# voidstrike/FPSG

Hardware: AMD Instinct MI355X
Metric: episodes/sec (+ Chamfer-kernel HBM GB/s in roofline.hbm), 2048-pt clouds, 224x224 images; episode = fwd + Chamfer + bwd, step = E episodes + all-reduce + Adam (higher is better)
Workload: dtype f32

## Files before the change

fpsg_amd/_hip.py:

```python
from __future__ import annotations

import ctypes
import os
import threading

import torch

_HERE = os.path.dirname(os.path.abspath(__file__))
LIB_PATH = os.environ.get("FPSG_HIP_LIB") or os.path.join(_HERE, "libfpsg_hip.so")

_c_f32p = ctypes.c_void_p
_c_i32p = ctypes.c_void_p
_c_int = ctypes.c_int
_c_stream = ctypes.c_void_p

SIGNATURES = {
    "fpsg_version": [],
    "fpsg_last_error": [],
    "fpsg_stream_threshold_bytes": [],
    "fpsg_chamfer_fwd": [_c_f32p, _c_f32p, _c_int, _c_int, _c_int,
                         _c_f32p, _c_i32p, _c_f32p, _c_i32p, _c_stream],
    "fpsg_chamfer_bwd": [_c_f32p, _c_f32p, _c_i32p, _c_i32p, _c_f32p, _c_f32p,
                         _c_int, _c_int, _c_int, _c_f32p, _c_f32p, _c_stream],
    "fpsg_chamfer_losses": [_c_f32p, _c_f32p, _c_int, _c_int, _c_int, _c_int, ctypes.c_float, ctypes.c_float, _c_f32p,
# ... 73 lines not shown
                             _c_f32p, _c_f32p, _c_f32p, _c_f32p, _c_stream],
    "fpsg_bn_act_bwd_parts": [_c_f32p, _c_f32p, _c_f32p, _c_f32p, _c_int, _c_int, _c_int, _c_int, _c_int,
                        ctypes.c_float, _c_f32p, _c_f32p, _c_f32p, _c_f32p, _c_f32p, _c_f32p, _c_f32p, _c_int, _c_stream],
    "fpsg_bn_pool_workspace_floats": [_c_int, _c_int, _c_int, _c_int],
    "fpsg_bn_act_pool_fwd": [_c_f32p, _c_f32p, _c_f32p, _c_f32p, _c_f32p, _c_f32p, ctypes.c_float, _c_int, _c_int, _c_int, _c_int,
                             _c_int, ctypes.c_float, _c_int, ctypes.c_float, _c_f32p, _c_f32p, _c_f32p, _c_f32p,
                             _c_f32p, _c_f32p, _c_int, _c_stream],
    "fpsg_bn_act_pool_bwd": [_c_f32p, _c_f32p, _c_f32p, _c_f32p, _c_int, _c_int, _c_int, _c_int, _c_int, _c_int,
                             ctypes.c_float, _c_f32p, _c_f32p, _c_f32p, _c_f32p, _c_f32p, _c_f32p, _c_stream],
    "fpsg_bn_max_workspace_floats": [_c_int, _c_int, _c_int],
    "fpsg_bn_max_dz_offset": [_c_int, _c_int, _c_int],
    "fpsg_bn_act_max_fwd": [_c_f32p, _c_f32p, _c_f32p, _c_f32p, _c_f32p, _c_f32p, ctypes.c_float, _c_int, _c_int, _c_int, _c_int,
                            ctypes.c_float, _c_int, ctypes.c_float, _c_f32p, _c_i32p, _c_f32p, _c_f32p, _c_f32p,
                            _c_f32p, _c_stream],
    "fpsg_bn_act_max_bwd": [_c_f32p, _c_f32p, _c_f32p, _c_i32p, _c_f32p, _c_int, _c_int, _c_int, _c_int, _c_int,
                            ctypes.c_float, _c_f32p, _c_f32p, _c_f32p, _c_f32p, _c_f32p, _c_f32p, _c_stream],
    "fpsg_max_bwd_prep": [_c_f32p, _c_f32p, _c_f32p, _c_f32p, _c_f32p, _c_f32p, _c_int, _c_int, _c_int, _c_int, _c_f32p, _c_f32p,
                          _c_f32p, _c_f32p, _c_stream],
    "fpsg_max_bwd_dw": [_c_f32p, _c_f32p, _c_f32p, _c_f32p, _c_f32p, _c_int, _c_int, _c_int, _c_f32p, _c_stream],
    "fpsg_max_bwd_gather": [_c_f32p, _c_f32p, _c_i32p, _c_int, _c_int, _c_int, _c_int, _c_f32p, _c_f32p, _c_stream],
    "fpsg_max_bwd_scatter": [_c_f32p, _c_f32p, _c_f32p, _c_f32p, _c_i32p, _c_f32p, _c_int, _c_int, _c_int, _c_int, _c_f32p,
                             _c_stream],
    "fpsg_max_bwd_scatter_workspace_floats": [_c_int, _c_int, _c_int],
    "fpsg_bn_act_max_bwd_coef": [_c_f32p, _c_f32p, _c_f32p, _c_i32p, _c_f32p, _c_int, _c_int, _c_int, _c_int, _c_int,
                                 ctypes.c_float, _c_f32p, _c_f32p, _c_f32p, _c_f32p, _c_stream],
    "fpsg_wino_input_transform": [_c_int, _c_f32p, _c_int, _c_int, _c_int, _c_int, _c_f32p, ctypes.c_long, _c_stream],
    "fpsg_wino_output_transform": [_c_int, _c_f32p, _c_int, _c_int, _c_int, _c_int, _c_f32p, ctypes.c_long, _c_stream],
    "fpsg_wino_stats_parts": [_c_int, _c_int, _c_int, _c_int],
    "fpsg_wino_output_transform_stats": [_c_int, _c_f32p, _c_int, _c_int, _c_int, _c_int, _c_f32p, _c_f32p, _c_f32p,
                                         ctypes.c_long, _c_stream],
    "fpsg_wino_grad_output_transform": [_c_int, _c_f32p, _c_int, _c_int, _c_int, _c_int, _c_f32p, ctypes.c_long, _c_stream],
    "fpsg_wino_grad_transforms": [_c_int, _c_f32p, _c_int, _c_int, _c_int, _c_int, _c_f32p, _c_f32p, ctypes.c_long, _c_stream],
    "fpsg_wino_filter_transform": [_c_int, _c_f32p, _c_int, _c_int, _c_int, _c_f32p, _c_stream],
    "fpsg_wino_output_transform_bwd_stats": [_c_int, _c_f32p, _c_int, _c_int, _c_int, _c_int, _c_f32p, _c_f32p, _c_f32p,
                                             _c_f32p, _c_f32p, ctypes.c_long, _c_stream],
    "fpsg_wino_filter_transform_batch": [ctypes.c_void_p, _c_int, ctypes.c_long, _c_stream],
    "fpsg_wino_filter_grad_transform": [_c_int, _c_f32p, _c_int, _c_int, _c_f32p, _c_stream],
    "fpsg_wino_conv_fused": [_c_f32p, _c_f32p, _c_int, _c_int, _c_int, _c_int, _c_int, _c_f32p, _c_stream],
    "fpsg_wino_input_transform_act": [_c_int, _c_f32p, _c_f32p, _c_f32p, _c_int, _c_int, _c_int, _c_int, _c_f32p, ctypes.c_long,
                                      _c_stream],
    "fpsg_wino_conv_fused_act": [_c_f32p, _c_f32p, _c_f32p, _c_f32p, _c_int, _c_int, _c_int, _c_int, _c_int, _c_f32p,
                                 _c_stream],
    "fpsg_wino_dw_fused_workspace_floats": [_c_int, _c_int, _c_int, _c_int],
    "fpsg_wino_dw_fused": [_c_f32p, _c_f32p, _c_f32p, _c_f32p, _c_int, _c_int, _c_int, _c_int, _c_int, _c_f32p, _c_f32p,
                           _c_stream],
    "fpsg_wino_conv_fused_parts": [_c_int, _c_int, _c_int, _c_int],
    "fpsg_wino_conv_fused_stats": [_c_f32p, _c_f32p, _c_f32p, _c_f32p, _c_int, _c_int, _c_int, _c_int, _c_int, _c_f32p,
                                   _c_f32p, _c_f32p, _c_stream],
    "fpsg_bn_stats": [_c_f32p, _c_f32p, _c_f32p, _c_f32p, _c_f32p, _c_f32p, ctypes.c_float, _c_int, _c_int, _c_int, _c_int,
                      ctypes.c_float, _c_f32p, _c_f32p, _c_f32p, _c_f32p, _c_f32p, _c_int, _c_stream],
    "fpsg_conv_first_dw_workspace_floats": [_c_int, _c_int, _c_int],
    "fpsg_conv_first_parts": [_c_int, _c_int, _c_int],
    "fpsg_conv_first_fwd": [_c_f32p, _c_f32p, _c_int, _c_int, _c_int, _c_int, _c_int, _c_f32p, _c_f32p, _c_f32p, _c_stream],
    "fpsg_conv_first_dw": [_c_f32p, _c_f32p, _c_int, _c_int, _c_int, _c_int, _c_int, _c_f32p, _c_f32p, _c_stream],
    "fpsg_conv_first_dw_fold": [_c_f32p, _c_f32p, _c_f32p, _c_f32p, _c_f32p, _c_f32p, _c_int, _c_int, _c_int, _c_int, _c_int,
                                _c_f32p, _c_f32p, _c_stream],
    "fpsg_adam_step": [_c_f32p, _c_f32p, _c_f32p, _c_f32p, ctypes.c_size_t, ctypes.c_float, ctypes.c_float,
                       ctypes.c_float, ctypes.c_float, _c_int, ctypes.c_float, _c_stream],
    "fpsg_flat_accumulate_segments": [_c_f32p, ctypes.c_void_p, ctypes.c_void_p, _c_int, ctypes.c_size_t, _c_int, _c_stream],
    "fpsg_flat_accumulate_tables": [_c_f32p, ctypes.c_void_p, ctypes.c_void_p, _c_int, _c_int, ctypes.c_size_t, _c_int,
                                    _c_stream],
    "fpsg_adam_step_segments": [_c_f32p, ctypes.c_void_p, ctypes.c_void_p, _c_int, _c_f32p, _c_f32p, ctypes.c_size_t,
                                ctypes.c_float, ctypes.c_float, ctypes.c_float, ctypes.c_float, _c_int, ctypes.c_float,
                                _c_stream],
    "fpsg_grad_norm_workspace_bytes": [ctypes.c_size_t],
    "fpsg_grad_clip_scale": [_c_f32p, ctypes.c_size_t, ctypes.c_float, ctypes.c_float, ctypes.c_void_p, ctypes.c_size_t,
# ... 180 lines not shown
```

fpsg_amd/csrc/winograd.hip:

```cpp
#include "fpsg_common.h"

namespace fpsg {
namespace {

template <bool NT>
__device__ __forceinline__ void stream_store(float* p, float v) {
  if constexpr (NT) __builtin_nontemporal_store(v, p);
  else *p = v;
}
template <bool NT>
__device__ __forceinline__ float stream_load(const float* p) {
  if constexpr (NT) return __builtin_nontemporal_load(p);
  else return *p;
}

constexpr int kWinoThreads = 256;

template <int M> struct Wino;

template <> struct Wino<2> {
  static constexpr int A = 4;
  static __device__ __forceinline__ void in(const float (&d)[4], float (&t)[4]) {
    t[0] = d[0] - d[2]; t[1] = d[1] + d[2]; t[2] = d[2] - d[1]; t[3] = d[1] - d[3];
  }
// ... 318 lines not shown
      v2 lo = {0.0f, 0.0f}, hi = {0.0f, 0.0f};
      if (M * ti.th + i < H) {
        lo = *reinterpret_cast<const v2*>(yp + (size_t)i * W);
        if (M * ti.tw + 2 < W) hi = *reinterpret_cast<const v2*>(yp + (size_t)i * W + 2);
      }
      yv[i][0] = lo[0]; yv[i][1] = lo[1]; yv[i][M - 2] = hi[0]; yv[i][M - 1] = hi[1];
    } else {
      const vin v = *reinterpret_cast<const vin*>(yp + (size_t)i * W);
#pragma unroll
      for (int j = 0; j < M; ++j) yv[i][j] = v[j];
    }
  }
  float r[M][A];
#pragma unroll
  for (int j = 0; j < M; ++j) {
    float col[M];
#pragma unroll
    for (int i = 0; i < M; ++i) col[i] = yv[i][j];
    Wino<M>::gout(col, r[j]);
  }
  const size_t plane = (size_t)K * Ps;
  float* mp = dM + (size_t)k * Ps + p;
#pragma unroll
  for (int i = 0; i < A; ++i) {
    float row[M], o[A];
#pragma unroll
    for (int j = 0; j < M; ++j) row[j] = r[j][i];
    Wino<M>::gout(row, o);
#pragma unroll
    for (int j = 0; j < A; ++j) stream_store<NT>(mp + (size_t)(A * i + j) * plane, o[j]);
  }
}

template <int M>
__device__ __forceinline__ void wino_filter_one(const float* __restrict__ w, int K, int C, int flip, float* __restrict__ U,
                                                long e) {
  constexpr int A = Wino<M>::A;
  const int k = flip ? (int)(e % K) : (int)(e / C), c = flip ? (int)(e / K) : (int)(e % C);
  const float* g = w + ((size_t)k * C + c) * 9;
  float t[3][A];
#pragma unroll
  for (int j = 0; j < 3; ++j) {
    float col[3];
#pragma unroll
    for (int i = 0; i < 3; ++i) col[i] = flip ? g[(2 - i) * 3 + (2 - j)] : g[i * 3 + j];
    Wino<M>::flt(col, t[j]);
  }
  const size_t plane = (size_t)K * C;
  float* up = U + (flip ? (size_t)c * K + k : (size_t)k * C + c);
#pragma unroll
  for (int i = 0; i < A; ++i) {
    float row[3], o[A];
#pragma unroll
    for (int j = 0; j < 3; ++j) row[j] = t[j][i];
    Wino<M>::flt(row, o);
#pragma unroll
    for (int j = 0; j < A; ++j) up[(size_t)(A * i + j) * plane] = o[j];
  }
}

template <int M>
__global__ void wino_filter_kernel(const float* __restrict__ w, int K, int C, int flip, float* __restrict__ U) {
  const long e = (long)blockIdx.x * blockDim.x + threadIdx.x;
  if (e >= (long)K * C) return;
  wino_filter_one<M>(w, K, C, flip, U, e);
}
// ... 210 lines not shown
                                          fpsg_stream_t stream) {
  using namespace fpsg;
  FPSG_REQUIRE(m == 2 || m == 4, FPSG_E_SHAPE, "fpsg_wino_filter_transform: m must be 2 or 4 (got %d)", m);
  FPSG_REQUIRE(K > 0 && C > 0, FPSG_E_SHAPE, "fpsg_wino_filter_transform: K,C must be positive (got %d,%d)", K, C);
  FPSG_REQUIRE_PTR(w); FPSG_REQUIRE_PTR(U);
  const long n = (long)K * C;
  dim3 grid((unsigned)((n + 255) / 256));
  if (m == 2) hipLaunchKernelGGL(wino_filter_kernel<2>, grid, dim3(256), 0, static_cast<hipStream_t>(stream), w, K, C, flip_transpose, U);
  else hipLaunchKernelGGL(wino_filter_kernel<4>, grid, dim3(256), 0, static_cast<hipStream_t>(stream), w, K, C, flip_transpose, U);
  return launch_status("fpsg_wino_filter_transform");
}

extern "C" int fpsg_wino_filter_transform_batch(const int64_t* jobs, int n_jobs, long total_blocks, fpsg_stream_t stream) {
  using namespace fpsg;
  FPSG_REQUIRE(n_jobs > 0 && total_blocks > 0 && total_blocks < (1L << 31), FPSG_E_SHAPE,
               "fpsg_wino_filter_transform_batch: n_jobs and total_blocks must be positive (got %d, %ld)", n_jobs, total_blocks);
  FPSG_REQUIRE_PTR(jobs);
  hipLaunchKernelGGL(wino_filter_batch_kernel, dim3((unsigned)total_blocks), dim3(256), 0, static_cast<hipStream_t>(stream),
                     reinterpret_cast<const long long*>(jobs), n_jobs);
  return launch_status("fpsg_wino_filter_transform_batch");
}

extern "C" int fpsg_wino_filter_grad_transform(int m, const float* dU, int K, int C, float* dw, fpsg_stream_t stream) {
  using namespace fpsg;
  FPSG_REQUIRE(m == 2 || m == 4, FPSG_E_SHAPE, "fpsg_wino_filter_grad_transform: m must be 2 or 4 (got %d)", m);
  FPSG_REQUIRE(K > 0 && C > 0, FPSG_E_SHAPE, "fpsg_wino_filter_grad_transform: K,C must be positive (got %d,%d)", K, C);
  FPSG_REQUIRE_PTR(dU); FPSG_REQUIRE_PTR(dw);
  const long n = (long)K * C;
  dim3 grid((unsigned)((n + 255) / 256));
  if (m == 2) hipLaunchKernelGGL(wino_filter_grad_kernel<2>, grid, dim3(256), 0, static_cast<hipStream_t>(stream), dU, K, C, dw);
  else hipLaunchKernelGGL(wino_filter_grad_kernel<4>, grid, dim3(256), 0, static_cast<hipStream_t>(stream), dU, K, C, dw);
  return launch_status("fpsg_wino_filter_grad_transform");
}
```

fpsg_amd/winograd.py:

```python
from __future__ import annotations

import os

import torch

from . import _hip, gemm_split
from .bn_counters import count_batch

MIN_CHANNELS_M4 = 64
MIN_CHANNELS_M2 = 128
MIN_WIDE_CHANNELS_M2 = 256


def enabled() -> bool:
    return os.environ.get("FPSG_WINOGRAD", "1") != "0"


def _eligible_layer(conv: torch.nn.Conv2d, H: int, W: int) -> bool:
    def is_(v, want):
        return v == want or v == (want, want)
    return (enabled() and is_(conv.kernel_size, 3) and is_(conv.stride, 1) and is_(conv.padding, 1) and is_(conv.dilation, 1)
            and conv.groups == 1 and conv.padding_mode == "zeros" and H % 2 == 0 and W % 2 == 0
            and _wide_enough(conv.in_channels, conv.out_channels, tile_size(H, W)))

# ... 213 lines not shown
    if dev.type != "cuda" or torch.cuda.is_current_stream_capturing():
        return chan, 0
    opt = lambda t: _hip.ptr(t) if t is not None else None
    with torch.cuda.device(dev):
        _call("fpsg_bn_stats", _hip.ptr(chan), None, opt(gamma), opt(beta), _hip.ptr(running_mean), _hip.ptr(running_var),
              0.0, 1, C, 1, 0, float(eps), _hip.ptr(chan), None, None, None, None, 0,
              torch.cuda.current_stream(dev).cuda_stream)
    cache[key] = chan
    return chan, 2


def _filter(m, w, flip):
    key = (w.data_ptr(), m, bool(flip))
    capturing = w.is_cuda and torch.cuda.is_current_stream_capturing()
    banked = _bank.lookup(key, w, capturing)
    if banked is not None:
        return banked
    cache = _frozen_cache
    if cache is not None and capturing:
        cache = _ReadOnlyView(cache) if _frozen_constant else None
    if cache is not None and key in cache:
        return cache[key]
    K, C = w.shape[0], w.shape[1]
    a2 = (m + 2) ** 2
    U = torch.empty((a2, C, K) if flip else (a2, K, C), dtype=torch.float32, device=w.device)
    _call("fpsg_wino_filter_transform", m, _hip.ptr(w), K, C, 1 if flip else 0, _hip.ptr(U), _hip.stream_of(w))
    if cache is not None and not capturing:
        cache[key] = U
        if filter_bank_enabled():
            _bank.register(key, w.detach(), U)
    return U


def row_stride(P: int) -> int:
    a = int(os.environ.get("FPSG_WINO_ROW_ALIGN", "32"))
    if a < 1 or a > 1024:
        raise ValueError(f"FPSG_WINO_ROW_ALIGN must be in 1 .. 1024 (got {a})")
    return (P + a - 1) // a * a


def _ldp(T, N, H, W, m):
    if not T.is_contiguous() or T.shape[2] < N * _tiles(H, W, m):
        raise ValueError(f"transform-domain tensor {tuple(T.shape)} must be contiguous with at least "
                         f"{N * _tiles(H, W, m)} columns")
    return T.shape[2]


def _input(m, x):
    N, C, H, W = x.shape
    Ps = row_stride(N * _tiles(H, W, m))
    V = torch.empty(((m + 2) ** 2, C, Ps), dtype=torch.float32, device=x.device)
    _call("fpsg_wino_input_transform", m, _hip.ptr(x), N, C, H, W, _hip.ptr(V), Ps, _hip.stream_of(x))
    return V


def stats_enabled() -> bool:
    return os.environ.get("FPSG_CONV_STATS", "1") != "0"


_BN_SMALL_MAX = 16384


def bwd_stats_enabled() -> bool:
    return os.environ.get("FPSG_CONV_BWD_STATS", "1") != "0"


# ... 30 lines not shown
    opt = lambda t: _hip.ptr(t) if t is not None else None
    _call("fpsg_wino_conv_fused_stats", _hip.ptr(x), opt(chan), opt(pre_bias), _hip.ptr(U), N, C, K, H, W, _hip.ptr(y),
          opt(stats_bias), _hip.ptr(parts), _hip.stream_of(x))
    return y, parts


def _fused(x, U):
    N, C, H, W = x.shape
    K = U.shape[1]
    y = torch.empty((N, K, H, W), dtype=torch.float32, device=x.device)
    _call("fpsg_wino_conv_fused", _hip.ptr(x), _hip.ptr(U), N, C, K, H, W, _hip.ptr(y), _hip.stream_of(x))
    return y


def _grad_output(m, gy):
    N, K, H, W = gy.shape
    Ps = row_stride(N * _tiles(H, W, m))
    dM = torch.empty(((m + 2) ** 2, K, Ps), dtype=torch.float32, device=gy.device)
    _call("fpsg_wino_grad_output_transform", m, _hip.ptr(gy), N, K, H, W, _hip.ptr(dM), Ps, _hip.stream_of(gy))
    return dM


def grad_transforms_enabled() -> bool:
    return os.environ.get("FPSG_GRAD_TRANSFORMS", "1") != "0"


def _grad_transforms(m, gy):
    N, K, H, W = gy.shape
    Ps = row_stride(N * _tiles(H, W, m))
    V = torch.empty(((m + 2) ** 2, K, Ps), dtype=torch.float32, device=gy.device)
    dM = torch.empty_like(V)
    _call("fpsg_wino_grad_transforms", m, _hip.ptr(gy), N, K, H, W, _hip.ptr(V), _hip.ptr(dM), Ps, _hip.stream_of(gy))
    return V, dM


def _filter_grad(m, dU, like):
    gw = torch.empty_like(like)
    _call("fpsg_wino_filter_grad_transform", m, _hip.ptr(dU), like.shape[0], like.shape[1], _hip.ptr(gw),
          _hip.stream_of(dU))
    return gw


class _Conv3x3(torch.autograd.Function):

    @staticmethod
    def forward(ctx, x, w, m, stats_bias=None, want_parts=False):
        ctx.set_materialize_grads(False)
        x, w = x.contiguous(), w.contiguous()
        N, C, H, W = x.shape
        K = w.shape[0]
        parts = None
        with torch.cuda.device(x.device):
            if _can_fuse(m, C, K, N * H * W, H, W):
                if want_parts:
                    y, parts = _fused_stats(x, None, None, _filter(m, w, False), stats_bias)
                else:
                    y = _fused(x, _filter(m, w, False))
                keep, kept_is_v = x, False
            else:
                V = _input(m, x)
                Mt = _bmm(_filter(m, w, False), V)
                if want_parts:
                    y, parts = _output(m, Mt, N, H, W, stats_bias, True)
                else:
                    y = _output(m, Mt, N, H, W)
                keep, kept_is_v = V, True
        ctx.save_for_backward(keep if ctx.needs_input_grad[1] else None, w)
        ctx.dims = (N, C, H, W, m, kept_is_v)
        if not want_parts:
            return y
        if parts is not None:
            ctx.mark_non_differentiable(parts)
        return y, parts

    @staticmethod
    def backward(ctx, gy, _gparts=None):
        if gy is None:
            return None, None, None, None, None
        kept, w = ctx.saved_tensors
        N, C, H, W, m, kept_is_v = ctx.dims
        K = w.shape[0]
        gy = gy.contiguous()
        gx = gw = None
        with torch.cuda.device(gy.device):
            fuse_dx = _can_fuse(m, K, C, N * H * W, H, W)
            fuse_dw = not kept_is_v and _can_fuse_dw(m, C, K, N, H, W)
            Vg = dM = None
            if (ctx.needs_input_grad[0] and ctx.needs_input_grad[1] and not fuse_dx and not fuse_dw
                    and grad_transforms_enabled()):
                Vg, dM = _grad_transforms(m, gy)
            if ctx.needs_input_grad[0]:
                if fuse_dx:
                    gx = _fused(gy, _filter(m, w, True))
                else:
                    gx = _output(m, _bmm(_filter(m, w, True), Vg if Vg is not None else _input(m, gy)), N, H, W)
                    Vg = None
            if ctx.needs_input_grad[1]:
                if fuse_dw:
                    gw = _filter_grad(m, _fused_dw(kept, None, None, gy), w)
                else:
                    V = kept if kept_is_v else _input(m, kept)
                    gw = _filter_grad(m, _bmm_nt(dM if dM is not None else _grad_output(m, gy), V), w)
        return gx, gw, None, None, None


def _input_act(m, x, chan, pre_bias):
    N, C, H, W = x.shape
    Ps = row_stride(N * _tiles(H, W, m))
    V = torch.empty(((m + 2) ** 2, C, Ps), dtype=torch.float32, device=x.device)
    _call("fpsg_wino_input_transform_act", m, _hip.ptr(x), _hip.ptr(chan), _hip.ptr(pre_bias) if pre_bias is not None else None,
          N, C, H, W, _hip.ptr(V), Ps, _hip.stream_of(x))
    return V


def _fused_act(x, chan, pre_bias, U):
    N, C, H, W = x.shape
    K = U.shape[1]
    y = torch.empty((N, K, H, W), dtype=torch.float32, device=x.device)
    _call("fpsg_wino_conv_fused_act", _hip.ptr(x), _hip.ptr(chan), _hip.ptr(pre_bias) if pre_bias is not None else None,
          _hip.ptr(U), N, C, K, H, W, _hip.ptr(y), _hip.stream_of(x))
    return y


def fold_enabled() -> bool:
    return os.environ.get("FPSG_BN_FOLD", "1") != "0"
# ... 29 lines not shown
                    out = _fused_act(y, chan, pre_bias, _filter(m, w, False))
                V = None
            else:
                V = _input_act(m, y, chan, pre_bias)
                Mt = _bmm(_filter(m, w, False), V)
                if want_parts:
                    out, out_parts = _output(m, Mt, N, H, W, stats_bias, True)
                else:
                    out = _output(m, Mt, N, H, W)
        ctx.save_for_backward(y, chan, pre_bias, w, V if ctx.needs_input_grad[9] else None)
        ctx.cfg = (N, C, H, W, m, bool(training), gamma is not None, beta is not None)
        if not want_parts:
            return out
        if out_parts is not None:
            ctx.mark_non_differentiable(out_parts)
        return out, out_parts

    @staticmethod
    def backward(ctx, gout, _gparts=None):
        if gout is None:
            return (None,) * 14
        y, chan, pre_bias, w, V = ctx.saved_tensors
        N, C, H, W, m, training, has_g, has_b = ctx.cfg
        K = w.shape[0]
        lib = _hip.load()
        dev = y.device
        gout = gout.contiguous()
        gw = None
        with torch.cuda.device(dev):
            bwd_parts = None
            fuse_dx = _can_fuse(m, K, C, N * H * W, H, W)
            fuse_dw = V is None and _can_fuse_dw(m, C, K, N, H, W)
            Vg = dM = None
            if ctx.needs_input_grad[9] and not fuse_dx and not fuse_dw and grad_transforms_enabled():
                Vg, dM = _grad_transforms(m, gout)
            if fuse_dx:
                ga = _fused(gout, _filter(m, w, True))
            elif bwd_stats_enabled() and N * H * W > _BN_SMALL_MAX:
                ga, bwd_parts = _output_bwd_stats(m, _bmm(_filter(m, w, True), Vg if Vg is not None else _input(m, gout)),
                                                  N, H, W, y, pre_bias, chan)
            else:
                ga = _output(m, _bmm(_filter(m, w, True), Vg if Vg is not None else _input(m, gout)), N, H, W)
            Vg = None
            if ctx.needs_input_grad[9]:
                if fuse_dw:
                    gw = _filter_grad(m, _fused_dw(y, chan, pre_bias, gout), w)
                else:
                    if V is None:
                        V = _input_act(m, y, chan, pre_bias)
                    gw = _filter_grad(m, _bmm_nt(dM if dM is not None else _grad_output(m, gout), V), w)
            want_dpb = pre_bias is not None and ctx.needs_input_grad[1]
            dy = torch.empty_like(y)
            dgamma = torch.empty((C,), dtype=torch.float32, device=dev)
            dbeta = torch.empty((C,), dtype=torch.float32, device=dev)
            dpb = torch.empty((C,), dtype=torch.float32, device=dev) if want_dpb else None
            coef = torch.empty((3, C), dtype=torch.float32, device=dev)
            ws = torch.empty((lib.fpsg_bn_workspace_floats(N, C, H * W),), dtype=torch.float32, device=dev)
            if bwd_parts is not None:
                _call("fpsg_bn_act_bwd_parts", _hip.ptr(y), _hip.ptr(pre_bias) if pre_bias is not None else None,
                      _hip.ptr(ga), _hip.ptr(chan), N, C, H * W, 1 if training else 0, 1, 0.0, _hip.ptr(dy),
                      _hip.ptr(dgamma), _hip.ptr(dbeta), _hip.ptr(dpb) if want_dpb else None, _hip.ptr(coef),
                      _hip.ptr(ws), _hip.ptr(bwd_parts), bwd_parts.shape[1], _hip.stream_of(y))
            else:
                _call("fpsg_bn_act_bwd", _hip.ptr(y), _hip.ptr(pre_bias) if pre_bias is not None else None, _hip.ptr(ga),
                      _hip.ptr(chan), N, C, H * W, 1 if training else 0, 1, 0.0, _hip.ptr(dy), _hip.ptr(dgamma),
                      _hip.ptr(dbeta), _hip.ptr(dpb) if want_dpb else None, _hip.ptr(coef), _hip.ptr(ws), _hip.stream_of(y))
        return (dy, dpb, dgamma if has_g else None, dbeta if has_b else None, None, None, None, None, None, gw, None,
                None, None, None)

# ... 129 lines not shown
```

include/fpsg_hip.h:

```cpp
#ifndef FPSG_HIP_H
#define FPSG_HIP_H

#include <stddef.h>
#include <stdint.h>

#ifdef __cplusplus
extern "C" {
#endif

typedef void* fpsg_stream_t;

#define FPSG_ABI_VERSION 1

#define FPSG_E_NULL   (-1)
#define FPSG_E_SHAPE  (-2)
#define FPSG_E_ALIGN  (-3)
#define FPSG_E_LIMIT  (-4)

int         fpsg_version(void);
const char* fpsg_last_error(void);
size_t      fpsg_stream_threshold_bytes(void);

int fpsg_chamfer_fwd(const float* xyz1, const float* xyz2, int B, int N, int M,
                     float* dist1, int32_t* idx1, float* dist2, int32_t* idx2,
// ... 235 lines not shown
int fpsg_bn_act_max_bwd(const float* x, const float* pre_bias, const float* gout, const int32_t* idx,
                        const float* chan, int N, int C, int L, int training, int act, float slope, float* dx,
                        float* dgamma, float* dbeta, float* dpre_bias, float* coef, float* ws, fpsg_stream_t stream);
int fpsg_bn_act_max_bwd_coef(const float* x, const float* pre_bias, const float* gout, const int32_t* idx,
                             const float* chan, int N, int C, int L, int training, int act, float slope,
                             float* dgamma, float* dbeta, float* coef, float* ws, fpsg_stream_t stream);

int fpsg_max_bwd_gather(const float* a, const float* dz, const int32_t* idx, int B, int K, int C, int L, float* S,
                        float* spart , fpsg_stream_t stream);
int fpsg_max_bwd_prep(const float* W, const float* coef, const float* pre_bias, const float* mean, const float* dz,
                      const float* spart, int B, int K, int C, int L, float* Wk, float* u, float* dpre_bias, float* s,
                      fpsg_stream_t stream);
int fpsg_max_bwd_dw(const float* S, const float* WG, const float* coef, const float* pre_bias, const float* s, int B,
                    int K, int C, float* dw, fpsg_stream_t stream);
size_t fpsg_max_bwd_scatter_workspace_floats(int B, int C, int L);
int fpsg_max_bwd_scatter(float* da, const float* W, const float* k1, const float* dz, const int32_t* idx, const float* v,
                         int B, int K, int C, int L, float* ws, fpsg_stream_t stream);


int fpsg_wino_input_transform(int m, const float* x, int N, int C, int H, int W, float* V, long ldp,
                              fpsg_stream_t stream);
int fpsg_wino_output_transform(int m, const float* M, int N, int K, int H, int W, float* y, long ldp,
                               fpsg_stream_t stream);
int fpsg_wino_stats_parts(int m, int N, int H, int W);
int fpsg_wino_output_transform_stats(int m, const float* M, int N, int K, int H, int W, float* y, const float* bias,
                                     float* parts, long ldp, fpsg_stream_t stream);
int fpsg_wino_output_transform_bwd_stats(int m, const float* M, int N, int K, int H, int W, float* y,
                                         const float* xpre, const float* pre_bias, const float* chan,
                                         float* parts, long ldp, fpsg_stream_t stream);
int fpsg_wino_grad_output_transform(int m, const float* dy, int N, int K, int H, int W, float* dM, long ldp,
                                    fpsg_stream_t stream);
int fpsg_wino_grad_transforms(int m, const float* dy, int N, int K, int H, int W, float* V, float* dM, long ldp,
                              fpsg_stream_t stream);
int fpsg_wino_filter_transform(int m, const float* w, int K, int C, int flip_transpose, float* U,
                               fpsg_stream_t stream);
int fpsg_wino_filter_transform_batch(const int64_t* jobs, int n_jobs, long total_blocks, fpsg_stream_t stream);
int fpsg_wino_filter_grad_transform(int m, const float* dU, int K, int C, float* dw, fpsg_stream_t stream);

size_t fpsg_gemm_split_workspace_floats(int batch, int M, int N, int K, int transB, int variant);
int fpsg_gemm_split(const float* A, const float* B, float* C, int batch, int M, int N, int K, int lda, int ldb, int ldc,
                    long sA, long sB, long sC, int transB, int variant, float* ws, size_t ws_floats,
                    fpsg_stream_t stream);

size_t fpsg_gemm_split_packed_a_bytes(int batch, int M, int K, int variant);
int fpsg_gemm_split_pack_a(const float* A, int batch, int M, int K, int lda, long sA, int variant, void* Ap,
                           fpsg_stream_t stream);
int fpsg_gemm_split_nn_packed(const void* Ap, const float* B, float* C, int batch, int M, int N, int K, int ldb, int ldc,
                              long sB, long sC, int variant, fpsg_stream_t stream);

int fpsg_gemm_split_nn_persistent(const void* Ap, const float* B, float* C, int batch, int M, int N, int K, int ldb, int ldc,
                                  long sB, long sC, int variant, fpsg_stream_t stream);

int fpsg_gemm_f32_nn(const float* A, const float* B, float* C, int batch, int M, int N, int K, int lda, int ldb, int ldc,
                     long sA, long sB, long sC, int variant, fpsg_stream_t stream);

int fpsg_wino_conv_fused(const float* x, const float* U, int N, int C, int K, int H, int W, float* y,
                         fpsg_stream_t stream);

int fpsg_wino_conv_fused_parts(int N, int K, int H, int W);
int fpsg_wino_conv_fused_stats(const float* x, const float* chan, const float* pre_bias, const float* U, int N, int C,
                               int K, int H, int W, float* y, const float* out_bias, float* parts, fpsg_stream_t stream);

size_t fpsg_wino_dw_fused_workspace_floats(int N, int K, int H, int W);
int fpsg_wino_dw_fused(const float* x, const float* chan, const float* pre_bias, const float* dy, int N, int C, int K,
                       int H, int W, float* dU, float* ws, fpsg_stream_t stream);

// ... 129 lines not shown
```

Baseline: 45.85.

## Compute Winograd conv input gradient via adjoint of input transform

For F(4x4,3x3) Winograd convolutions, the data gradient is now computed as the transpose of the forward: the output gradient is grad-output-transformed (dM), multiplied by a transposed filter transform, then scattered back through the adjoint of the input transform. Overlapping tile contributions are handled with neighbour loads and wave shuffles, and a variant fuses the BN/activation backward statistics. This avoids re-running the input transform on the output gradient and the separate flipped-filter path, reusing dM that dw already needs. It applies only for large tensors (>=64MB transform buffer) and adds a more complex halo-handling kernel.

Measured after the change: 46.40 (median of 2 runs). No clear change (+1.2%).

```diff
diff --git a/fpsg_amd/_hip.py b/fpsg_amd/_hip.py
--- a/fpsg_amd/_hip.py
+++ b/fpsg_amd/_hip.py
@@ -129,6 +129,10 @@
     "fpsg_wino_grad_output_transform": [_c_int, _c_f32p, _c_int, _c_int, _c_int, _c_int, _c_f32p, ctypes.c_long, _c_stream],
     "fpsg_wino_grad_transforms": [_c_int, _c_f32p, _c_int, _c_int, _c_int, _c_int, _c_f32p, _c_f32p, ctypes.c_long, _c_stream],
     "fpsg_wino_filter_transform": [_c_int, _c_f32p, _c_int, _c_int, _c_int, _c_f32p, _c_stream],
+    "fpsg_wino_input_adjoint_parts": [_c_int, _c_int, _c_int],
+    "fpsg_wino_input_adjoint": [_c_int, _c_f32p, _c_int, _c_int, _c_int, _c_int, ctypes.c_long, _c_f32p, _c_stream],
+    "fpsg_wino_input_adjoint_bwd_stats": [_c_int, _c_f32p, _c_int, _c_int, _c_int, _c_int, ctypes.c_long, _c_f32p, _c_f32p,
+                                          _c_f32p, _c_f32p, _c_f32p, _c_int, _c_stream],
     "fpsg_wino_output_transform_bwd_stats": [_c_int, _c_f32p, _c_int, _c_int, _c_int, _c_int, _c_f32p, _c_f32p, _c_f32p,
                                              _c_f32p, _c_f32p, ctypes.c_long, _c_stream],
     "fpsg_wino_filter_transform_batch": [ctypes.c_void_p, _c_int, ctypes.c_long, _c_stream],
diff --git a/fpsg_amd/csrc/winograd.hip b/fpsg_amd/csrc/winograd.hip
--- a/fpsg_amd/csrc/winograd.hip
+++ b/fpsg_amd/csrc/winograd.hip
@@ -374,6 +374,147 @@
   }
 }
 
+__device__ __forceinline__ void wino4_in_t(const float (&v)[6], float (&o)[6]) {
+  const float p12 = v[1] + v[2], m12 = v[1] - v[2], p34 = v[3] + v[4], m34 = v[3] - v[4];
+  o[0] = 4.0f * v[0];
+  o[1] = fma_rn(-4.0f, m12, fma_rn(-2.0f, m34, 4.0f * v[5]));
+  o[2] = fma_rn(-5.0f, v[0], fma_rn(-4.0f, p12, -p34));
+  o[3] = fma_rn(2.0f, m34, fma_rn(-5.0f, v[5], m12));
+  o[4] = (v[0] + p12) + p34;
+  o[5] = v[5];
+}
+
+template <bool NT, bool BWD>
+__global__ __launch_bounds__(kWinoThreads) void wino_input_adjoint_kernel(const float* __restrict__ dV, int C, int H, int W,
+                                                                           int Th, int Tw, long P, long Ps,
+                                                                           float* __restrict__ dx,
+                                                                           const float* __restrict__ xpre,
+                                                                           const float* __restrict__ pre_bias,
+                                                                           const float* __restrict__ chan,
+                                                                           float* __restrict__ parts) {
+  typedef float v4 __attribute__((ext_vector_type(4)));
+  const long p_raw = (long)blockIdx.x * kWinoThreads + threadIdx.x;
+  const bool live = p_raw < P;
+  const long p = live ? p_raw : P - 1;
+  const int c = blockIdx.y;
+  const TileIndex ti = tile_of(p, Th, Tw);
+  const int lane = threadIdx.x & (kWave - 1);
+  const bool has_left = ti.tw > 0, has_right = ti.tw < Tw - 1, has_up = ti.th > 0, has_down = ti.th < Th - 1;
+  const bool left_lane = has_left && lane > 0;
+  const bool right_lane = has_right && lane < kWave - 1;
+  const size_t plane = (size_t)C * Ps;
+  const float* vp = dV + (size_t)c * Ps + p;
+  const long up_off = has_up ? -(long)Tw : 0, dn_off = has_down ? (long)Tw : 0;
+  float own[36], up[6], dn[6];
+#pragma unroll
+  for (int q = 0; q < 36; ++q) own[q] = stream_load<NT>(vp + (size_t)q * plane);
+#pragma unroll
+  for (int j = 0; j < 6; ++j) {
+    up[j] = stream_load<NT>(vp + up_off + (size_t)(30 + j) * plane);
+    dn[j] = stream_load<NT>(vp + dn_off + (size_t)j * plane);
+  }
+  float el[8], er[8];
+#pragma unroll
+  for (int i = 0; i < 8; ++i) el[i] = er[i] = 0.0f;
+  if (has_left && !left_lane) {
+#pragma unroll
+    for (int i = 0; i < 6; ++i) el[i] = stream_load<NT>(vp - 1 + (size_t)(6 * i + 5) * plane);
+    el[6] = stream_load<NT>(vp - 1 + up_off + (size_t)35 * plane);
+    el[7] = stream_load<NT>(vp - 1 + dn_off + (size_t)5 * plane);
+  }
+  if (has_right && !right_lane) {
+#pragma unroll
+    for (int i = 0; i < 6; ++i) er[i] = stream_load<NT>(vp + 1 + (size_t)(6 * i) * plane);
+    er[6] = stream_load<NT>(vp + 1 + up_off + (size_t)30 * plane);
+    er[7] = stream_load<NT>(vp + 1 + dn_off);
+  }
+  const size_t yoff = (((size_t)ti.n * C + c) * H + 4 * ti.th) * W + 4 * ti.tw;
+  v4 xrow[4];
+  float b = 0.0f, sc = 0.0f, sh = 0.0f, mu = 0.0f, rs = 0.0f;
+  if constexpr (BWD) {
+    b = pre_bias ? pre_bias[c] : 0.0f;
+    sc = chan[c]; sh = chan[C + c]; mu = chan[2 * C + c]; rs = chan[3 * C + c];
+#pragma unroll
+    for (int i = 0; i < 4; ++i) xrow[i] = *reinterpret_cast<const v4*>(xpre + yoff + (size_t)i * W);
+  }
+  float t[6][6];
+#pragma unroll
+  for (int j = 0; j < 6; ++j) {
+    float col[6];
+#pragma unroll
+    for (int i = 0; i < 6; ++i) col[i] = own[6 * i + j];
+    wino4_in_t(col, t[j]);
+  }
+  float R[4][6];
+#pragma unroll
+  for (int i = 0; i < 4; ++i) {
+    float row[6];
+#pragma unroll
+    for (int j = 0; j < 6; ++j) row[j] = t[j][1 + i];
+    wino4_in_t(row, R[i]);
+  }
+  float u[6], d4[6], d[6];
+  wino4_in_t(up, u);
+#pragma unroll
+  for (int j = 0; j < 6; ++j) d4[j] = 4.0f * dn[j];
+  wino4_in_t(d4, d);
+#pragma unroll
+  for (int j = 0; j < 6; ++j) {
+    R[0][j] += has_up ? u[j] : 0.0f;
+    R[3][j] += has_down ? d[j] : 0.0f;
+  }
+  float lt[6], rt[6], L[4], Rr[4];
+  {
+    float lcol[6], rcol[6];
+#pragma unroll
+    for (int i = 0; i < 6; ++i) { lcol[i] = el[i]; rcol[i] = er[i]; }
+    wino4_in_t(lcol, lt);
+    wino4_in_t(rcol, rt);
+  }
+#pragma unroll
+  for (int i = 0; i < 4; ++i) { L[i] = lt[1 + i]; Rr[i] = 4.0f * rt[1 + i]; }
+  L[0] += has_up ? el[6] : 0.0f;
+  L[3] += has_down ? 4.0f * el[7] : 0.0f;
+  Rr[0] += has_up ? 4.0f * er[6] : 0.0f;
+  Rr[3] += has_down ? 4.0f * (4.0f * er[7]) : 0.0f;
+  float* yp = dx + yoff;
+  float a0 = 0.0f, a1 = 0.0f;
+#pragma unroll
+  for (int i = 0; i < 4; ++i) {
+    float lft = __shfl_up(R[i][5], 1, kWave);
+    float rgt = __shfl_down(R[i][0], 1, kWave);
+    if (!left_lane) lft = has_left ? L[i] : 0.0f;
+    if (!right_lane) rgt = has_right ? Rr[i] : 0.0f;
+    const float o[4] = {R[i][1] + lft, R[i][2], R[i][3], R[i][4] + rgt};
+    if (live) *reinterpret_cast<v4*>(yp + (size_t)i * W) = (v4){o[0], o[1], o[2], o[3]};
+    if constexpr (BWD) {
+#pragma unroll
+      for (int j = 0; j < 4; ++j) {
+        const float xv = xrow[i][j] + b;
+        const float dz = (live && fma_rn(xv, sc, sh) > 0.0f) ? o[j] : 0.0f;
+        a0 += dz;
+        a1 = fma_rn(dz, (xv - mu) * rs, a1);
+      }
+    }
+  }
+  if constexpr (BWD) {
+    __shared__ float red[2 * (kWinoThreads / kWave)];
+    a0 = wave_sum(a0);
+    a1 = wave_sum(a1);
+    const int wave = threadIdx.x / kWave;
+    if (lane == 0) { red[2 * wave] = a0; red[2 * wave + 1] = a1; }
+    __syncthreads();
+    if (threadIdx.x == 0) {
+      float t0 = red[0], t1 = red[1];
+#pragma unroll
+      for (int w = 1; w < kWinoThreads / kWave; ++w) { t0 += red[2 * w]; t1 += red[2 * w + 1]; }
+      float* out = parts + ((size_t)c * gridDim.x + blockIdx.x) * 2;
+      out[0] = t0;
+      out[1] = t1;
+    }
+  }
+}
+
 template <int M>
 __device__ __forceinline__ void wino_filter_one(const float* __restrict__ w, int K, int C, int flip, float* __restrict__ U,
                                                 long e) {
@@ -650,3 +791,67 @@
   else hipLaunchKernelGGL(wino_filter_grad_kernel<4>, grid, dim3(256), 0, static_cast<hipStream_t>(stream), dU, K, C, dw);
   return launch_status("fpsg_wino_filter_grad_transform");
 }
+
+namespace fpsg {
+namespace {
+
+int check_adjoint(const char* fn, int m, int N, int C, int H, int W, long ldp) {
+  FPSG_REQUIRE(m == 4, FPSG_E_SHAPE, "%s: m must be 4 (got %d)", fn, m);
+  FPSG_REQUIRE(N > 0 && C > 0 && H > 0 && W > 0 && H % 4 == 0 && W % 4 == 0, FPSG_E_SHAPE,
+               "%s: N,C positive and H,W positive multiples of 4 (got %d,%d,%d,%d)", fn, N, C, H, W);
+  const long P = (long)N * (H / 4) * (W / 4);
+  FPSG_REQUIRE(C <= 65535 && (P + kWinoThreads - 1) / kWinoThreads < (1L << 31), FPSG_E_LIMIT,
+               "%s: C=%d or tile count %ld beyond the grid limits", fn, C, P);
+  FPSG_REQUIRE(ldp == 0 || ldp >= P, FPSG_E_SHAPE, "%s: row stride %ld must be 0 or at least the %ld tiles", fn, ldp, P);
+  return 0;
+}
+
+}
+}
+
+extern "C" int fpsg_wino_input_adjoint_parts(int N, int H, int W) {
+  if (N <= 0 || H <= 0 || W <= 0 || H % 4 || W % 4) return 0;
+  const long P = (long)N * (H / 4) * (W / 4);
+  return (int)((P + fpsg::kWinoThreads - 1) / fpsg::kWinoThreads);
+}
+
+extern "C" int fpsg_wino_input_adjoint(int m, const float* dV, int N, int C, int H, int W, long ldp, float* dx,
+    fpsg_stream_t stream) {
+  using namespace fpsg;
+  int rc = check_adjoint("fpsg_wino_input_adjoint", m, N, C, H, W, ldp);
+  if (rc) return rc;
+  FPSG_REQUIRE_PTR(dV); FPSG_REQUIRE_PTR(dx);
+  FPSG_REQUIRE((reinterpret_cast<uintptr_t>(dx) & 15) == 0, FPSG_E_ALIGN, "fpsg_wino_input_adjoint: dx must be 16-byte aligned");
+  const int Th = H / 4, Tw = W / 4;
+  const long P = (long)N * Th * Tw;
+  const long Ps = ldp ? ldp : P;
+  dim3 grid((unsigned)((P + kWinoThreads - 1) / kWinoThreads), C);
+  hipStream_t hs = static_cast<hipStream_t>(stream);
+  if (beyond_cache((size_t)36 * C * Ps * sizeof(float))) hipLaunchKernelGGL((wino_input_adjoint_kernel<true, false>), grid, dim3(kWinoThreads), 0, hs, dV, C, H, W, Th, Tw, P, Ps, dx, nullptr, nullptr, nullptr, nullptr);
+  else hipLaunchKernelGGL((wino_input_adjoint_kernel<false, false>), grid, dim3(kWinoThreads), 0, hs, dV, C, H, W, Th, Tw, P, Ps, dx, nullptr, nullptr, nullptr, nullptr);
+  return launch_status("fpsg_wino_input_adjoint");
+}
+
+extern "C" int fpsg_wino_input_adjoint_bwd_stats(int m, const float* dV, int N, int C, int H, int W, long ldp, float* dx,
+                                                 const float* y, const float* pre_bias, const float* chan, float* parts,
+                                                 int n_parts,
+    fpsg_stream_t stream) {
+  using namespace fpsg;
+  int rc = check_adjoint("fpsg_wino_input_adjoint_bwd_stats", m, N, C, H, W, ldp);
+  if (rc) return rc;
+  FPSG_REQUIRE_PTR(dV); FPSG_REQUIRE_PTR(dx); FPSG_REQUIRE_PTR(y); FPSG_REQUIRE_PTR(chan); FPSG_REQUIRE_PTR(parts);
+  FPSG_REQUIRE(((reinterpret_cast<uintptr_t>(dx) | reinterpret_cast<uintptr_t>(y)) & 15) == 0, FPSG_E_ALIGN,
+               "fpsg_wino_input_adjoint_bwd_stats: dx and y must be 16-byte aligned");
+  FPSG_REQUIRE(!misaligned4(pre_bias), FPSG_E_ALIGN, "fpsg_wino_input_adjoint_bwd_stats: pre_bias not 4-byte aligned");
+  const int Th = H / 4, Tw = W / 4;
+  const long P = (long)N * Th * Tw;
+  const long Ps = ldp ? ldp : P;
+  FPSG_REQUIRE(n_parts == fpsg_wino_input_adjoint_parts(N, H, W), FPSG_E_SHAPE,
+               "fpsg_wino_input_adjoint_bwd_stats: n_parts %d must be fpsg_wino_input_adjoint_parts(N,H,W) = %d", n_parts,
+               fpsg_wino_input_adjoint_parts(N, H, W));
+  dim3 grid((unsigned)((P + kWinoThreads - 1) / kWinoThreads), C);
+  hipStream_t hs = static_cast<hipStream_t>(stream);
+  if (beyond_cache((size_t)36 * C * Ps * sizeof(float))) hipLaunchKernelGGL((wino_input_adjoint_kernel<true, true>), grid, dim3(kWinoThreads), 0, hs, dV, C, H, W, Th, Tw, P, Ps, dx, y, pre_bias, chan, parts);
+  else hipLaunchKernelGGL((wino_input_adjoint_kernel<false, true>), grid, dim3(kWinoThreads), 0, hs, dV, C, H, W, Th, Tw, P, Ps, dx, y, pre_bias, chan, parts);
+  return launch_status("fpsg_wino_input_adjoint_bwd_stats");
+}
diff --git a/fpsg_amd/winograd.py b/fpsg_amd/winograd.py
--- a/fpsg_amd/winograd.py
+++ b/fpsg_amd/winograd.py
@@ -269,6 +269,23 @@
     return U
 
 
+def _filter_t(m, w):
+    key = (w.data_ptr(), m, "t")
+    capturing = w.is_cuda and torch.cuda.is_current_stream_capturing()
+    cache = _frozen_cache
+    if cache is not None and capturing:
+        cache = _ReadOnlyView(cache) if _frozen_constant else None
+    if cache is not None and key in cache:
+        return cache[key]
+    K, C = w.shape[0], w.shape[1]
+    wt = w.transpose(0, 1).contiguous()
+    U = torch.empty(((m + 2) ** 2, C, K), dtype=torch.float32, device=w.device)
+    _call("fpsg_wino_filter_transform", m, _hip.ptr(wt), C, K, 0, _hip.ptr(U), _hip.stream_of(w))
+    if cache is not None and not capturing:
+        cache[key] = U
+    return U
+
+
 def row_stride(P: int) -> int:
     a = int(os.environ.get("FPSG_WINO_ROW_ALIGN", "32"))
     if a < 1 or a > 1024:
@@ -365,6 +382,34 @@
     dM = torch.empty_like(V)
     _call("fpsg_wino_grad_transforms", m, _hip.ptr(gy), N, K, H, W, _hip.ptr(V), _hip.ptr(dM), Ps, _hip.stream_of(gy))
     return V, dM
+
+
+MIN_ADJOINT_BYTES = 64 << 20
+
+
+def adjoint_mode() -> str:
+    return os.environ.get("FPSG_WINO_ADJOINT", "auto")
+
+
+def _adjoint_applies(m: int, K: int, N: int, H: int, W: int) -> bool:
+    mode = adjoint_mode()
+    if mode == "0" or m != 4 or H % 4 or W % 4:
+        return False
+    return mode == "1" or 36 * K * row_stride(N * _tiles(H, W, 4)) * 4 >= MIN_ADJOINT_BYTES
+
+
+def _input_adjoint(m, dV, N, H, W, xpre=None, pre_bias=None, chan=None):
+    C = dV.shape[1]
+    ga = torch.empty((N, C, H, W), dtype=torch.float32, device=dV.device)
+    if xpre is None:
+        _call("fpsg_wino_input_adjoint", m, _hip.ptr(dV), N, C, H, W, _ldp(dV, N, H, W, m), _hip.ptr(ga), _hip.stream_of(dV))
+        return ga
+    S = _hip.load().fpsg_wino_input_adjoint_parts(N, H, W)
+    parts = torch.empty((C, S, 2), dtype=torch.float32, device=dV.device)
+    _call("fpsg_wino_input_adjoint_bwd_stats", m, _hip.ptr(dV), N, C, H, W, _ldp(dV, N, H, W, m), _hip.ptr(ga),
+          _hip.ptr(xpre), _hip.ptr(pre_bias) if pre_bias is not None else None, _hip.ptr(chan), _hip.ptr(parts), S,
+          _hip.stream_of(dV))
+    return ga, parts
 
 
 def _filter_grad(m, dU, like):
@@ -419,11 +464,16 @@
             fuse_dx = _can_fuse(m, K, C, N * H * W, H, W)
             fuse_dw = not kept_is_v and _can_fuse_dw(m, C, K, N, H, W)
             Vg = dM = None
-            if (ctx.needs_input_grad[0] and ctx.needs_input_grad[1] and not fuse_dx and not fuse_dw
-                    and grad_transforms_enabled()):
+            both = ctx.needs_input_grad[0] and ctx.needs_input_grad[1] and not fuse_dx and not fuse_dw
+            adjoint = both and _adjoint_applies(m, K, N, H, W)
+            if adjoint:
+                dM = _grad_output(m, gy)
+            elif both and grad_transforms_enabled():
                 Vg, dM = _grad_transforms(m, gy)
             if ctx.needs_input_grad[0]:
-                if fuse_dx:
+                if adjoint:
+                    gx = _input_adjoint(m, _bmm(_filter_t(m, w), dM), N, H, W)
+                elif fuse_dx:
                     gx = _fused(gy, _filter(m, w, True))
                 else:
                     gx = _output(m, _bmm(_filter(m, w, True), Vg if Vg is not None else _input(m, gy)), N, H, W)
@@ -519,9 +569,20 @@
             fuse_dx = _can_fuse(m, K, C, N * H * W, H, W)
             fuse_dw = V is None and _can_fuse_dw(m, C, K, N, H, W)
             Vg = dM = None
-            if ctx.needs_input_grad[9] and not fuse_dx and not fuse_dw and grad_transforms_enabled():
+            both = ctx.needs_input_grad[9] and not fuse_dx and not fuse_dw
+            adjoint = both and _adjoint_applies(m, K, N, H, W)
+            if adjoint:
+                dM = _grad_output(m, gout)
+            elif both and grad_transforms_enabled():
                 Vg, dM = _grad_transforms(m, gout)
-            if fuse_dx:
+            if adjoint:
+                dV = _bmm(_filter_t(m, w), dM)
+                if bwd_stats_enabled() and N * H * W > _BN_SMALL_MAX:
+                    ga, bwd_parts = _input_adjoint(m, dV, N, H, W, y, pre_bias, chan)
+                else:
+                    ga = _input_adjoint(m, dV, N, H, W)
+                dV = None
+            elif fuse_dx:
                 ga = _fused(gout, _filter(m, w, True))
             elif bwd_stats_enabled() and N * H * W > _BN_SMALL_MAX:
                 ga, bwd_parts = _output_bwd_stats(m, _bmm(_filter(m, w, True), Vg if Vg is not None else _input(m, gout)),
diff --git a/include/fpsg_hip.h b/include/fpsg_hip.h
--- a/include/fpsg_hip.h
+++ b/include/fpsg_hip.h
@@ -291,6 +291,12 @@
                                     fpsg_stream_t stream);
 int fpsg_wino_grad_transforms(int m, const float* dy, int N, int K, int H, int W, float* V, float* dM, long ldp,
                               fpsg_stream_t stream);
+int fpsg_wino_input_adjoint_parts(int N, int H, int W);
+int fpsg_wino_input_adjoint(int m, const float* dV, int N, int C, int H, int W, long ldp, float* dx,
+                            fpsg_stream_t stream);
+int fpsg_wino_input_adjoint_bwd_stats(int m, const float* dV, int N, int C, int H, int W, long ldp, float* dx,
+                                      const float* y, const float* pre_bias, const float* chan, float* parts,
+                                      int n_parts, fpsg_stream_t stream);
 int fpsg_wino_filter_transform(int m, const float* w, int K, int C, int flip_transpose, float* U,
                                fpsg_stream_t stream);
 int fpsg_wino_filter_transform_batch(const int64_t* jobs, int n_jobs, long total_blocks, fpsg_stream_t stream);
```
